# loopinf/SpotV2Net

Measured on NVIDIA B200. Metric: SpotV2Net GAT fwd+bwd graphs/sec (30-node, batch 4096), higher is better.
Workload: dtype f32

## Files before the change

spotv2net_b200/csrc/gemm.cuh:

```cuda
#pragma once
#include "common.cuh"

namespace spotv2 {

int sgemm_simt(bool a_kc, bool b_kc, int M, int N, int K, const float* A, int lda, const float* B,
               int ldb, float* C, int ldc, int splits, void* ws, size_t ws_bytes, cudaStream_t st);

struct BGemm {
  int M, N, K;
  const float* A;
  const float* B;
  float* C;
  int lda, ldb, ldc;
  int inner;
  long long a_o, a_i, b_o, b_i, c_o, c_i;
  int segs;
  long long a_s, b_s;
  float scale;
  const float* bias;
  long long bias_i;
  int vecA, vecB;
  int tensor_cores;
};
int bgemm_simt(bool a_kc, bool b_kc, BGemm g, int batches, cudaStream_t st);

inline int weight_grad_splits(int rows, int m, int n) {
  int base = (rows + 8191) / 8192;
  if (base < 1) base = 1;
  if (base > 32) base = 32;
  if (base == 1) return 1;
  const int tiles = ((m + 127) / 128) * ((n + 255) / 256);
  int best = base;
  double best_eff = 0.0;
  for (int s = base; s <= base + base / 4 + 1 && s <= 32; ++s) {
    const int items = tiles * s;
    const double eff = (double)items / (double)(((items + 147) / 148) * 148);
    if (eff > best_eff + 1e-9) { best = s; best_eff = eff; }
  }
  return best;
}

bool tc_gemm_supported(bool a_kc, bool b_kc, int M, int N, int K, const float* A_hi, int lda, const float* B_hi, int ldb);
int split_tf32(const float* src, float* hi, float* lo, size_t n, cudaStream_t st);
int gemm3x_tf32(bool a_kc, bool b_kc, int M, int N, int K, const float* A_hi, const float* A_lo, int lda,
                const float* B_hi, const float* B_lo, int ldb, float* C, int ldc, int splits, int bn,
                int kb_per_chunk, void* ws, size_t ws_bytes, cudaStream_t st);

struct F16Operand {
  const void* hi;
  const void* lo;
  int ld;
  const float* inv;
  int split_at;
};
struct PairOut {
  void* hi;
  void* lo;
  int ld;
  const float* scale;
// ... 20 lines not shown
```

spotv2net_b200/csrc/gemm_f16.cu:

```cuda
#include <cuda_fp16.h>
#include <stdio.h>
#include <stdlib.h>
#include <string.h>

#include <algorithm>

#include "gemm.cuh"
#include "tc.cuh"
#include "tma.cuh"

namespace spotv2 {

namespace {

constexpr int HBM_ = 128;
constexpr int HUMMA_K = 16;
constexpr int kHThreads = 384;
constexpr int kHEpiWarps = 8;

struct HParams {
  int M, N, K;
  int ldc;
  float* C;
  int m_tiles, n_tiles, splits, kb_per_split, kb_total, kb_per_chunk;
  size_t split_stride;
  const float* a_inv;
  const float* b_inv;
  int a_split, b_split;
  int scale_in_kernel;
  unsigned* amax_out;
  int amax_cols;
  int single;
  int pair_out;
  const float* out_scale;
  float* tail32;
  int tail_ld;
  int tma_store;
  int dbg;
};
#ifdef SPOTV2_BRINGUP
#define SPOTV2_DBG(p) ((p).dbg)
#else
#define SPOTV2_DBG(p) 0
#endif

template <int BN, int TBK, bool A_KM, bool B_KM>
struct HSmem {
  static constexpr int kAOp = HBM_ * TBK * 2;
  static constexpr int kBOp = BN * TBK * 2;
  static constexpr int kStage = 2 * kAOp + 2 * kBOp;
  static constexpr bool kWideEpi = (TBK == 32) && A_KM && B_KM;
  static constexpr int kStages = kWideEpi ? 3 : ((200 * 1024) / kStage > 6 ? 6 : (200 * 1024) / kStage);
  static constexpr int kBarOff = kStages * kStage;
  static constexpr int kEpiOff = kBarOff + 1024;
  static constexpr int kEpiWarpBytes = kWideEpi ? 8192 : 32 * 33 * 4;
  static constexpr int kBoxStride = kWideEpi ? 8192 : 4096;
  static constexpr int kPairBoxes = kWideEpi ? 4 : 2;
  static constexpr int kEpiBytes = kHEpiWarps * kEpiWarpBytes;
  static constexpr int kTotal = kEpiOff + kEpiBytes + 1024;
  static constexpr uint32_t kTxBytes = kStage;
};

template <int BN, int TBK, bool A_KM, bool B_KM>
__global__ void __launch_bounds__(kHThreads, 1)
gemm3x_f16_kernel(const __grid_constant__ CUtensorMap tmAh, const __grid_constant__ CUtensorMap tmAl,
                  const __grid_constant__ CUtensorMap tmBh, const __grid_constant__ CUtensorMap tmBl,
                  const __grid_constant__ CUtensorMap tmC, const HParams p) {
  using S = HSmem<BN, TBK, A_KM, B_KM>;
  constexpr int kStages = S::kStages;
  extern __shared__ unsigned char smem_dyn[];
  unsigned char* smem = reinterpret_cast<unsigned char*>((reinterpret_cast<uintptr_t>(smem_dyn) + 1023) & ~uintptr_t(1023));
  uint64_t* full = reinterpret_cast<uint64_t*>(smem + S::kBarOff);
  uint64_t* empty = full + kStages;
  uint64_t* tfull = empty + kStages;
  uint64_t* tempty = tfull + 2;
  uint32_t* tmem_slot = reinterpret_cast<uint32_t*>(tempty + 2);

  const int warp = threadIdx.x >> 5, lane = threadIdx.x & 31;
  const int total_tiles = p.m_tiles * p.n_tiles * p.splits;
  constexpr uint32_t kTmemCols = 2 * BN;

  if (warp == 0 && lane == 0) {
    prefetch_tmap(&tmAh); prefetch_tmap(&tmAl); prefetch_tmap(&tmBh); prefetch_tmap(&tmBl);
  }
  if (warp == 1 && lane == 0) {
    for (int s = 0; s < kStages; ++s) { mbar_init(&full[s], 1); mbar_init(&empty[s], 1); }
    for (int s = 0; s < 2; ++s) { mbar_init(&tfull[s], 1); mbar_init(&tempty[s], kHEpiWarps); }
    fence_mbar_init();
  }
  if (warp == 2) tmem_alloc(tmem_slot, kTmemCols);
  tc_fence_before();
  __syncthreads();
  tc_fence_after();
  const uint32_t tmem_base = *tmem_slot;

  auto tile_coords = [&](int tile, int& mt, int& nt, int& sp) {
    nt = tile % p.n_tiles;
    const int r = tile / p.n_tiles;
    mt = r % p.m_tiles;
    sp = r / p.m_tiles;
  };

  if (warp == 0) {
    if (elect_one()) {
      int stage = 0; uint32_t phase = 0;
      for (int tile = blockIdx.x; tile < total_tiles; tile += gridDim.x) {
        int mt, nt, sp; tile_coords(tile, mt, nt, sp);
        const int kb0 = sp * p.kb_per_split;
        const int kb1 = min(p.kb_total, kb0 + p.kb_per_split);
        for (int kb = kb0; kb < kb1; ++kb) {
          mbar_wait(&empty[stage], phase ^ 1);
          unsigned char* st = smem + stage * S::kStage;
          const bool lo = !p.single;
          mbar_expect_tx(&full[stage], lo ? S::kTxBytes : S::kTxBytes / 2);
          const int k = kb * TBK;
          if (A_KM) {
            tma_load_2d(st, &tmAh, k, mt * HBM_, &full[stage]);
            if (lo) tma_load_2d(st + S::kAOp, &tmAl, k, mt * HBM_, &full[stage]);
          } else {
#pragma unroll
            for (int blk = 0; blk < HBM_ / 64; ++blk) {
              tma_load_2d(st + blk * (TBK * 128), &tmAh, mt * HBM_ + blk * 64, k, &full[stage]);
              if (lo) tma_load_2d(st + S::kAOp + blk * (TBK * 128), &tmAl, mt * HBM_ + blk * 64, k, &full[stage]);
            }
          }
          unsigned char* sb = st + 2 * S::kAOp;
          if (B_KM) {
            tma_load_2d(sb, &tmBh, k, nt * BN, &full[stage]);
            if (lo) tma_load_2d(sb + S::kBOp, &tmBl, k, nt * BN, &full[stage]);
          } else {
#pragma unroll
            for (int blk = 0; blk < BN / 64; ++blk) {
              tma_load_2d(sb + blk * (TBK * 128), &tmBh, nt * BN + blk * 64, k, &full[stage]);
              if (lo) tma_load_2d(sb + S::kBOp + blk * (TBK * 128), &tmBl, nt * BN + blk * 64, k, &full[stage]);
            }
          }
          if (++stage == kStages) { stage = 0; phase ^= 1; }
        }
      }
    }
  } else if (warp == 1) {
    if (elect_one()) {
      constexpr uint32_t idesc = (1u << 4) | ((A_KM ? 0u : 1u) << 15) | ((B_KM ? 0u : 1u) << 16) |
                                 ((uint32_t)(BN >> 3) << 17) | ((uint32_t)(HBM_ >> 4) << 24);
      constexpr uint32_t k_sbo = 8 * TBK * 2, k_lt = (TBK == 64) ? 2 : 4;
      constexpr uint32_t a_lbo = A_KM ? 16 : TBK * 128, b_lbo = B_KM ? 16 : TBK * 128;
      constexpr uint32_t a_sbo = A_KM ? k_sbo : 1024, b_sbo = B_KM ? k_sbo : 1024;
      constexpr uint32_t a_lt = A_KM ? k_lt : 2, b_lt = B_KM ? k_lt : 2;
      constexpr uint32_t a_kstep = A_KM ? HUMMA_K * 2 : HUMMA_K * 128;
      constexpr uint32_t b_kstep = B_KM ? HUMMA_K * 2 : HUMMA_K * 128;
      int stage = 0; uint32_t phase = 0;
      uint32_t chunk_ctr = 0;
      for (int tile = blockIdx.x; tile < total_tiles; tile += gridDim.x) {
        int mt, nt, sp; tile_coords(tile, mt, nt, sp);
        const int kb0 = sp * p.kb_per_split;
        const int kb1 = min(p.kb_total, kb0 + p.kb_per_split);
        for (int kc = kb0; kc < kb1; kc += p.kb_per_chunk, ++chunk_ctr) {
          const int as = chunk_ctr & 1;
          mbar_wait(&tempty[as], ((chunk_ctr >> 1) & 1) ^ 1);
          tc_fence_after();
          const uint32_t d_tmem = tmem_base + (uint32_t)(as * BN);
          uint32_t accum = 0;
          const int kce = min(kb1, kc + p.kb_per_chunk);
          for (int kb = kc; kb < kce; ++kb) {
            mbar_wait(&full[stage], phase);
            tc_fence_after();
            const uint32_t sa = smem_u32(smem + stage * S::kStage);
            const uint32_t sb = sa + 2 * S::kAOp;
#pragma unroll
            for (int ks = 0; ks < TBK / HUMMA_K; ++ks) {
              const uint64_t ah = make_desc(sa + ks * a_kstep, a_lbo, a_sbo, a_lt);
              const uint64_t al = make_desc(sa + S::kAOp + ks * a_kstep, a_lbo, a_sbo, a_lt);
              const uint64_t bh = make_desc(sb + ks * b_kstep, b_lbo, b_sbo, b_lt);
              const uint64_t bl = make_desc(sb + S::kBOp + ks * b_kstep, b_lbo, b_sbo, b_lt);
              if (!p.single) {
                umma_f16(d_tmem, al, bh, idesc, accum);
                umma_f16(d_tmem, ah, bl, idesc, 1);
                accum = 1;
              }
              umma_f16(d_tmem, ah, bh, idesc, accum);
              accum = 1;
            }
            umma_commit(&empty[stage]);
            if (++stage == kStages) { stage = 0; phase ^= 1; }
          }
          umma_commit(&tfull[as]);
        }
      }
    }
  } else if (warp >= 4) {
    constexpr int HALF = BN / 2;
    const int q = warp & 3;
    const int ch = (warp - 4) >> 2;
    uint32_t chunk_ctr = 0;
    for (int tile = blockIdx.x; tile < total_tiles; tile += gridDim.x) {
      int mt, nt, sp; tile_coords(tile, mt, nt, sp);
      const int kb0 = sp * p.kb_per_split;
      const int kb1 = min(p.kb_total, kb0 + p.kb_per_split);
      float acc[HALF];
#pragma unroll
      for (int e = 0; e < HALF; ++e) acc[e] = 0.f;
      for (int kc = kb0; kc < kb1; kc += p.kb_per_chunk, ++chunk_ctr) {
        const int as = chunk_ctr & 1;
        mbar_wait(&tfull[as], (chunk_ctr >> 1) & 1);
        tc_fence_after();
        const uint32_t taddr = tmem_base + ((uint32_t)(q * 32) << 16) + (uint32_t)(as * BN + ch * HALF);
#pragma unroll
        for (int c0 = 0; c0 < HALF; c0 += 32) {
          uint32_t r[32];
          tmem_ld32(taddr + c0, r);
#pragma unroll
          if (!(SPOTV2_DBG(p) & 4))
#pragma unroll
            for (int e = 0; e < 32; ++e) acc[c0 + e] += __uint_as_float(r[e]);
          else acc[c0] += __uint_as_float(r[0]);
        }
        tc_fence_before();
        __syncwarp();
        if (lane == 0) mbar_arrive(&tempty[as]);
      }
      const int row = mt * HBM_ + q * 32 + lane;
      const int col0 = nt * BN + ch * HALF;
      float row_amax = 0.f;
      if (row < p.M && col0 < p.N && !(SPOTV2_DBG(p) & 2)) {
        if (p.scale_in_kernel) {
          const float ra = p.a_inv ? p.a_inv[row >= p.a_split ? 1 : 0] : 1.f;
          const float os0 = p.pair_out ? p.out_scale[0] : 1.f, os1 = p.pair_out ? p.out_scale[1] : 1.f;
          const float cb0 = ra * (p.b_inv ? p.b_inv[0] : 1.f) * os0, cb1 = ra * (p.b_inv ? p.b_inv[1] : 1.f) * os1;
#pragma unroll
          for (int e = 0; e < HALF; ++e) acc[e] *= (col0 + e >= p.b_split) ? cb1 : cb0;
        }
        if (p.amax_out) {
          float mx = 0.f;
#pragma unroll
          for (int e = 0; e < HALF; ++e)
            if (col0 + e < p.amax_cols) mx = fmaxf(mx, fabsf(acc[e]));
          row_amax = mx;
        }
      }
      if (p.pair_out && p.tail32 && row < p.M && col0 + HALF > p.b_split && col0 < p.N) {
        const float un = 1.f / p.out_scale[1];
        float* dst = p.tail32 + (size_t)row * p.tail_ld - p.b_split;
// ... 68 lines not shown
#pragma unroll
        for (int cc = 0; cc < HALF / 32; ++cc) {
#pragma unroll
          for (int j = 0; j < 32; ++j) stage[lane * 33 + j] = acc[cc * 32 + j];
          __syncwarp();
          const int col = col0 + cc * 32 + lane;
          if (col < p.N) {
#pragma unroll 8
            for (int rr = 0; rr < 32; ++rr)
              if (row_base + rr < p.M) cbase[(size_t)rr * p.ldc + col] = stage[rr * 33 + lane];
          }
          __syncwarp();
        }
      }
      if (p.amax_out) {
        for (int o = 16; o > 0; o >>= 1) row_amax = fmaxf(row_amax, __shfl_xor_sync(0xffffffffu, row_amax, o));
        if (lane == 0 && row_amax > 0.f) atomicMax(p.amax_out, __float_as_uint(row_amax));
      }
    }
  }

  if (warp >= 4 && lane == 0) asm volatile("cp.async.bulk.wait_group 0;" ::: "memory");
  tc_fence_before();
  __syncthreads();
  if (warp == 2) {
    tc_fence_after();
    tmem_dealloc(tmem_base, kTmemCols);
  }
}

__global__ void f16_splitk_reduce_kernel(const float* __restrict__ ws, int splits, size_t split_stride, int M, int N,
                                         float* __restrict__ C, int ldc, const float* __restrict__ a_inv, int a_split,
                                         const float* __restrict__ b_inv, int b_split) {
  const size_t idx = (size_t)blockIdx.x * blockDim.x + threadIdx.x;
  if (idx >= (size_t)M * N) return;
  float s = 0.f;
  for (int z = 0; z < splits; ++z) s += ws[(size_t)z * split_stride + idx];
  const int m = (int)(idx / N), n = (int)(idx - (size_t)m * N);
  const float f = (a_inv ? a_inv[m >= a_split ? 1 : 0] : 1.f) * (b_inv ? b_inv[n >= b_split ? 1 : 0] : 1.f);
  C[(size_t)m * ldc + n] = s * f;
}

template <int BN, int TBK, bool A_KM, bool B_KM>
int launch_h(const CUtensorMap& tAh, const CUtensorMap& tAl, const CUtensorMap& tBh, const CUtensorMap& tBl,
             const CUtensorMap& tC, const HParams& p, cudaStream_t st) {
  using S = HSmem<BN, TBK, A_KM, B_KM>;
  auto kern = gemm3x_f16_kernel<BN, TBK, A_KM, B_KM>;
  SPOTV2_CUDA_OK(cudaFuncSetAttribute(kern, cudaFuncAttributeMaxDynamicSharedMemorySize, S::kTotal));
  int grid = sm_count();
  const int total = p.m_tiles * p.n_tiles * p.splits;
  if (grid > total) grid = total;
  kern<<<grid, kHThreads, S::kTotal, st>>>(tAh, tAl, tBh, tBl, tC, p);
  SPOTV2_CUDA_OK(cudaGetLastError());
  return SPOTV2_OK;
}

__device__ __forceinline__ float scale_from_amax(float amax) {
  if (!(amax > 0.f) || !(amax < INFINITY)) return 1.f;
  int ex;
  frexpf(amax, &ex);
  return exp2f((float)(15 - ex));
}

__global__ void amax_kernel(const float* __restrict__ src, int rows, int cols, size_t ld, int split_dim, int split_at,
                            const float* __restrict__ pre2, int pre_split, unsigned* __restrict__ out_bits) {
  float m0 = 0.f, m1 = 0.f;
  const size_t total = (size_t)rows * cols;
  for (size_t idx = (size_t)blockIdx.x * blockDim.x + threadIdx.x; idx < total; idx += (size_t)gridDim.x * blockDim.x) {
    const int r = (int)(idx / cols), c = (int)(idx - (size_t)r * cols);
    float v = fabsf(src[(size_t)r * ld + c]);
    if (pre2) v *= pre2[r >= pre_split ? 1 : 0];
    const bool g1 = (split_dim == 0 ? r : c) >= split_at;
    if (g1) m1 = fmaxf(m1, v); else m0 = fmaxf(m0, v);
  }
  for (int o = 16; o > 0; o >>= 1) {
    m0 = fmaxf(m0, __shfl_xor_sync(0xffffffffu, m0, o));
// ... 250 lines not shown
    } else {
      if (int rc = launch_amax_flat(src, (size_t)r_split * cols, bits, st)) return rc;
      if (r_split < rows)
        if (int rc = launch_amax_flat(src + (size_t)r_split * cols, (size_t)(rows - r_split) * cols, bits + 1, st)) return rc;
    }
  } else {
    amax_kernel<<<blocks, 256, 0, st>>>(src, rows, cols, ld, split_dim, split_at, pre2, pre_split, bits);
  }
  const int vec4 = (cols % 4 == 0) && (ld % 4 == 0) && (ld16 % 4 == 0) && aligned16(src) &&
                   ((reinterpret_cast<uintptr_t>(hi) & 7) == 0) && ((reinterpret_cast<uintptr_t>(lo) & 7) == 0);
  if (vec4 && cols / 4 < 64)
    split_f16_narrow_kernel<<<(unsigned)std::min<size_t>(((size_t)rows * (cols / 4) + 255) / 256, (size_t)16 * 148), 256, 0, st>>>(
        src, rows, cols / 4, ld, split_dim, split_at, pre2, pre_split, static_cast<__half*>(hi), static_cast<__half*>(lo), ld16, blk);
  else if (vec4)
    split_f16_rows_kernel<<<std::min((rows + kSplitRows - 1) / kSplitRows, 32 * 148), 256, 0, st>>>(
        src, rows, cols / 4, ld, split_dim, split_at, pre2, pre_split, static_cast<__half*>(hi), static_cast<__half*>(lo), ld16, blk);
  else
    split_f16_kernel<<<blocks, 256, 0, st>>>(src, rows, cols, ld, split_dim, split_at, pre2, pre_split, 1.f,
                                             static_cast<__half*>(hi), static_cast<__half*>(lo), ld16, blk, 0);
  SPOTV2_CUDA_OK(cudaGetLastError());
  return SPOTV2_OK;
}

int gemm3x_f16(bool a_kc, bool b_kc, int M, int N, int K, const F16Operand& A, const F16Operand& B, float* C, int ldc,
               int splits, int bn, int kb_per_chunk, void* ws, size_t ws_bytes, cudaStream_t st, float* amax_out,
               int amax_cols, bool single, const PairOut* pair) {
  const int TBK = (bn & 16) ? 32 : 64;
  bn &= ~16;
  if (!tma_available()) return fail(SPOTV2_ERR_NO_DEVICE, "tensor-core GEMM: TMA descriptor encoding is not available");
  if (A.ld % 8 != 0 || B.ld % 8 != 0 || !aligned16(A.hi) || !aligned16(A.lo) || !aligned16(B.hi) || !aligned16(B.lo))
    return fail(SPOTV2_ERR_INVALID_ARG, "fp16 GEMM operands need 16-byte aligned bases and leading dimensions % 8 == 0");
  HParams p;
  p.M = M; p.N = N; p.K = K;
  p.m_tiles = (M + HBM_ - 1) / HBM_;
  p.n_tiles = (N + bn - 1) / bn;
  p.kb_total = (K + TBK - 1) / TBK;
  if (splits < 1) splits = 1;
  if (splits > p.kb_total) splits = p.kb_total;
  p.kb_per_split = (p.kb_total + splits - 1) / splits;
  p.splits = (p.kb_total + p.kb_per_split - 1) / p.kb_per_split;
  p.kb_per_chunk = kb_per_chunk < 1 ? 128 / TBK : kb_per_chunk;
  p.C = C; p.ldc = ldc; p.split_stride = 0;
  p.a_inv = A.inv; p.b_inv = B.inv; p.a_split = A.split_at; p.b_split = B.split_at;
  p.scale_in_kernel = 1;
  p.amax_out = reinterpret_cast<unsigned*>(amax_out);
  p.amax_cols = amax_cols;
  p.single = single ? 1 : 0;
  p.pair_out = 0; p.out_scale = nullptr; p.tail32 = nullptr; p.tail_ld = 0;
  if (pair) {
    if (splits > 1 || !pair->hi || !pair->scale || pair->ld % 8 != 0 || !aligned16(pair->hi) || (pair->lo && !aligned16(pair->lo)))
      return fail(SPOTV2_ERR_INVALID_ARG, "gemm3x_f16: pair output needs splits == 1, 16-byte aligned planes, ld %% 8 == 0 and a scale");
    p.pair_out = pair->lo ? 1 : 2;
    p.out_scale = pair->scale;
    p.tail32 = pair->tail32; p.tail_ld = pair->tail_ld;
  }
  p.dbg = 0;
#ifdef SPOTV2_BRINGUP
// ... 25 lines not shown
  if (pair) {
    const uint64_t plane_stride = pair->lo ? (uint64_t)((const __half*)pair->lo - (const __half*)pair->hi) : (uint64_t)M * pair->ld;
    if (pair->lo && ((const __half*)pair->lo <= (const __half*)pair->hi || plane_stride % 8 != 0))
      return fail(SPOTV2_ERR_INVALID_ARG, "gemm3x_f16: the lo plane must follow the hi plane at a multiple of 16 bytes");
    if ((rc = make_tmap3_f16(&tC, pair->hi, pair->lo ? 2 : 1, plane_stride, (uint64_t)M, (uint64_t)N, (uint64_t)pair->ld, 32, 32,
                             CU_TENSOR_MAP_SWIZZLE_64B)))
      return rc;
  } else if (aligned16(p.C) && p.ldc % 4 == 0 && (p.splits == 1 || p.split_stride % 4 == 0)) {
    if ((rc = make_tmap3(&tC, p.C, (uint64_t)p.splits, p.splits > 1 ? p.split_stride : (uint64_t)M * p.ldc, (uint64_t)M, (uint64_t)N,
                         (uint64_t)p.ldc, 16, 32, CU_TENSOR_MAP_SWIZZLE_64B)))
      return rc;
    p.tma_store = 1;
  }
  const CUtensorMapSwizzle kSw = TBK == 64 ? CU_TENSOR_MAP_SWIZZLE_128B : CU_TENSOR_MAP_SWIZZLE_64B;
  const CUtensorMapSwizzle mnSw = CU_TENSOR_MAP_SWIZZLE_128B;
  if (a_kc) {
    if ((rc = make_tmap_f16(&tAh, A.hi, M, K, A.ld, TBK, HBM_, kSw))) return rc;
    if ((rc = make_tmap_f16(&tAl, A.lo, M, K, A.ld, TBK, HBM_, kSw))) return rc;
  } else {
    if ((rc = make_tmap_f16(&tAh, A.hi, K, M, A.ld, 64, TBK, mnSw))) return rc;
    if ((rc = make_tmap_f16(&tAl, A.lo, K, M, A.ld, 64, TBK, mnSw))) return rc;
  }
  if (b_kc) {
    if ((rc = make_tmap_f16(&tBh, B.hi, N, K, B.ld, TBK, bn, kSw))) return rc;
    if ((rc = make_tmap_f16(&tBl, B.lo, N, K, B.ld, TBK, bn, kSw))) return rc;
  } else {
    if ((rc = make_tmap_f16(&tBh, B.hi, K, N, B.ld, 64, TBK, mnSw))) return rc;
    if ((rc = make_tmap_f16(&tBl, B.lo, K, N, B.ld, 64, TBK, mnSw))) return rc;
  }
#define SPOTV2_H(BN_, TBK_, AK, BK_) rc = launch_h<BN_, TBK_, AK, BK_>(tAh, tAl, tBh, tBl, tC, p, st)
#define SPOTV2_H_MAJ(BN_, TBK_)                            \
  do {                                                     \
    if (a_kc && b_kc) SPOTV2_H(BN_, TBK_, true, true);     \
    else if (a_kc) SPOTV2_H(BN_, TBK_, true, false);       \
    else if (b_kc) SPOTV2_H(BN_, TBK_, false, true);       \
    else SPOTV2_H(BN_, TBK_, false, false);                \
  } while (0)
  if (bn == 256 && TBK == 64) SPOTV2_H_MAJ(256, 64);
  else if (bn == 256 && TBK == 32) SPOTV2_H_MAJ(256, 32);
  else if (bn == 128 && TBK == 64) SPOTV2_H_MAJ(128, 64);
  else return fail(SPOTV2_ERR_INVALID_ARG, "bn must be 128, 256 or 256+16");
#undef SPOTV2_H_MAJ
#undef SPOTV2_H
  if (rc) return rc;
  if (p.splits > 1) {
    const size_t total = (size_t)M * N;
    f16_splitk_reduce_kernel<<<(unsigned)((total + 255) / 256), 256, 0, st>>>(p.C, p.splits, p.split_stride, M, N, C, ldc,
                                                                             A.inv, A.split_at, B.inv, B.split_at);
    SPOTV2_CUDA_OK(cudaGetLastError());
  }
  return SPOTV2_OK;
}

// ... 2 lines not shown
```

spotv2net_b200/csrc/proj.cu:

```cuda
#include "attn_bwd.cuh"
#include "gemm.cuh"

using namespace spotv2;

namespace {

constexpr int kNone = 0x7fffffff;

struct ProjShape {
  int rows, n_aug, HC, F, ldp, ldf16, ldp16;
};

ProjShape shape_of(const spotv2_gat_desc* d) {
  const int n_aug = n_aug_of(d);
  return {d->B * d->N, n_aug, d->H * head_pitch_of(d), d->F, d->ldp, ld16_of(d->F), ld16_of(n_aug)};
}

bool use_tc(const spotv2_gat_desc* d) { return d->gemm_algo != 1; }
bool single_product(const spotv2_gat_desc* d) { return d->gemm_algo == 3; }

struct Carver {
  unsigned char* p;
  size_t left;
  void* take(size_t bytes) {
// ... 1 lines not shown
    if (!p || bytes > left) return nullptr;
    void* r = p;
    p += bytes;
    left -= bytes;
    return r;
  }
};

size_t pair_bytes(size_t rows, size_t ld16) { return 2 * round_up(rows * ld16 * 2, 256); }

}

extern "C" int32_t spotv2_gat_ld16(int32_t cols) { return ld16_of(cols); }
extern "C" int32_t spotv2_diag_weight_grad_splits(int32_t rows, int32_t m, int32_t n) { return weight_grad_splits(rows, m, n); }

extern "C" int spotv2_gat_workspace_bytes(const spotv2_gat_desc* d, size_t* proj_fwd,
                                          size_t* attn_bwd, size_t* proj_bwd) {
  if (int rc = check_desc(d)) return rc;
  const ProjShape s = shape_of(d);
  const bool tc = use_tc(d);
  if (proj_fwd) *proj_fwd = 1024 + (tc ? pair_bytes(s.rows, s.ldf16) + pair_bytes(s.n_aug, s.ldf16) : 0);
  if (attn_bwd) *attn_bwd = attn_bwd_ws_bytes(d) + 256;
  if (proj_bwd) {
    const int splits = weight_grad_splits(s.rows, s.n_aug, s.F);
    size_t w = round_up((size_t)splits * s.n_aug * s.F * sizeof(float), 256) + 1024;
    if (tc) w += pair_bytes(s.rows, s.ldp16) + pair_bytes(s.rows, s.ldf16) + pair_bytes(s.n_aug, s.ldf16);
    *proj_bwd = w;
  }
  return SPOTV2_OK;
}

extern "C" int spotv2_gat_attn_fwd_workspace_bytes(const spotv2_gat_desc* d, size_t* attn_fwd) {
  if (int rc = check_desc(d)) return rc;
  SPOTV2_REQUIRE(attn_fwd, "attn_fwd_workspace_bytes: null pointer");
  *attn_fwd = attn_large_fwd_ws_bytes(d);
  return SPOTV2_OK;
}

extern "C" int spotv2_gat_edge_terms_bytes(const spotv2_gat_desc* d, size_t* bytes) {
  if (int rc = check_desc(d)) return rc;
  SPOTV2_REQUIRE(bytes, "edge_terms_bytes: null pointer");
  const size_t per_graph = (size_t)d->H * d->N * (d->N > 32 ? (size_t)d->N : (size_t)kEdgeTermNS);
  *bytes = d->Fe > 0 ? (size_t)d->B * per_graph * sizeof(float) : 0;
  return SPOTV2_OK;
}

extern "C" int spotv2_gat_uses_tensor_cores(const spotv2_gat_desc* d) {
// ... 52 lines not shown
  cudaStream_t st = as_stream(stream);
  Carver c{static_cast<unsigned char*>(ws), ws ? ws_bytes : 0};
  float* wblk = static_cast<float*>(c.take(2 * kScaleBlockFloats * sizeof(float)));
  void* wh = c.take((size_t)s.n_aug * s.ldf16 * 2);
  void* wl = c.take((size_t)s.n_aug * s.ldf16 * 2);
  if (!wblk || !wh || !wl) return fail(SPOTV2_ERR_WORKSPACE, "proj_fwd_pair: workspace too small (%zu B)", ws_bytes);
  if (int rc = w_pair_and_out_scale(W_aug, s.n_aug, s.F, s.HC, wh, wl, s.ldf16, wblk, x_scale, p_scale, st)) return rc;
  F16Operand A{x_hi, x_lo, s.ldf16, x_scale + 2, kNone}, B{wh, wl, s.ldf16, wblk + 2, s.HC};
  PairOut out{P_hi, single_product(d) ? nullptr : P_lo_or_null, s.ldp16, p_scale + 4, sd, 2 * d->H};
  return gemm3x_f16(true, true, s.rows, s.n_aug, s.F, A, B, nullptr, 0, 1, 256 + 16, 0, nullptr, 0, st, nullptr, 0, single_product(d),
                    &out);
}

extern "C" int spotv2_proj_bwd_weight(const spotv2_gat_desc* d, const float* x, const void* x_hi, const void* x_lo,
                                      const float* x_scale, const float* dP_aug, const void* dP_hi, const void* dP_lo,
                                      const float* dp_scale, float* dW_aug, void* ws, size_t ws_bytes, void* stream) {
  if (int rc = check_desc(d)) return rc;
  SPOTV2_REQUIRE((x || x_hi) && dW_aug && (dP_aug || dP_hi), "proj_bwd_weight: null pointer");
  if (d->p_format == 1 && single_product(d) && dP_hi && !dP_lo) dP_lo = dP_hi;
  SPOTV2_REQUIRE(d->p_format == 0 || (dP_hi && dP_lo && dp_scale && x_hi && x_lo && x_scale),
                 "proj_bwd_weight: p_format 1 takes x and dP as pairs");
  const ProjShape s = shape_of(d);
  cudaStream_t st = as_stream(stream);
  const int splits = weight_grad_splits(s.rows, s.n_aug, s.F);
  if (!use_tc(d)) {
    SPOTV2_REQUIRE(dP_aug, "proj_bwd_weight: the CUDA-core path takes the fp32 dP_aug");
    return sgemm_simt(false, false, s.n_aug, s.F, s.rows, dP_aug, s.ldp, x, s.F, dW_aug, s.F, splits, ws, ws_bytes, st);
  }
  Carver c{static_cast<unsigned char*>(ws), ws ? ws_bytes : 0};
  float* blk = static_cast<float*>(c.take(2 * kScaleBlockFloats * sizeof(float)));
  const bool have_x = x_hi && x_lo && x_scale, have_p = dP_hi && dP_lo && dp_scale;
  void* ph = have_p ? const_cast<void*>(dP_hi) : c.take((size_t)s.rows * s.ldp16 * 2);
  void* pl = have_p ? const_cast<void*>(dP_lo) : c.take((size_t)s.rows * s.ldp16 * 2);
  void* xh = have_x ? const_cast<void*>(x_hi) : c.take((size_t)s.rows * s.ldf16 * 2);
  void* xl = have_x ? const_cast<void*>(x_lo) : c.take((size_t)s.rows * s.ldf16 * 2);
  if (!blk || !ph || !pl || !xh || !xl) return fail(SPOTV2_ERR_WORKSPACE, "proj_bwd_weight: workspace too small (%zu B)", ws_bytes);
  const float *ps = dp_scale, *xs = x_scale;
  if (!have_p) {
    SPOTV2_REQUIRE(dP_aug, "proj_bwd_weight: dP_aug or the complete pair (dP_hi, dP_lo, dp_scale)");
    if (int rc = split_f16(dP_aug, s.rows, s.n_aug, s.ldp, 1, s.HC, nullptr, 0, ph, pl, s.ldp16, blk, st)) return rc;
    ps = blk;
  }
  if (!have_x) {
    if (int rc = split_f16(x, s.rows, s.F, s.F, 0, kNone, nullptr, 0, xh, xl, s.ldf16, blk + kScaleBlockFloats, st)) return rc;
    xs = blk + kScaleBlockFloats;
  }
  F16Operand A{ph, pl, s.ldp16, ps + 2, s.HC}, B{xh, xl, s.ldf16, xs + 2, kNone};
// ... 38 lines not shown
```

spotv2net_b200/csrc/tc.cuh:

```cuda
#pragma once
#include "common.cuh"

namespace spotv2 {

__device__ __forceinline__ void mbar_arrive(uint64_t* bar) {
  asm volatile("mbarrier.arrive.shared::cta.b64 _, [%0];" ::"r"(smem_u32(bar)) : "memory");
}
__device__ __forceinline__ void tc_fence_before() { asm volatile("tcgen05.fence::before_thread_sync;" ::: "memory"); }
__device__ __forceinline__ void tc_fence_after() { asm volatile("tcgen05.fence::after_thread_sync;" ::: "memory"); }
__device__ __forceinline__ void tmem_alloc(uint32_t* smem_dst, uint32_t ncols) {
  asm volatile("tcgen05.alloc.cta_group::1.sync.aligned.shared::cta.b32 [%0], %1;" ::"r"(smem_u32(smem_dst)), "r"(ncols)
               : "memory");
  asm volatile("tcgen05.relinquish_alloc_permit.cta_group::1.sync.aligned;" ::: "memory");
}
__device__ __forceinline__ void tmem_dealloc(uint32_t taddr, uint32_t ncols) {
  asm volatile("tcgen05.dealloc.cta_group::1.sync.aligned.b32 %0, %1;" ::"r"(taddr), "r"(ncols) : "memory");
}
__device__ __forceinline__ void umma_tf32(uint32_t tmem_d, uint64_t adesc, uint64_t bdesc, uint32_t idesc, uint32_t accum) {
  asm volatile(
      "{\n\t.reg .pred p;\n\tsetp.ne.b32 p, %4, 0;\n\t"
      "tcgen05.mma.cta_group::1.kind::tf32 [%0], %1, %2, %3, p;\n\t}" ::"r"(tmem_d),
      "l"(adesc), "l"(bdesc), "r"(idesc), "r"(accum)
      : "memory");
}
__device__ __forceinline__ void umma_f16(uint32_t tmem_d, uint64_t adesc, uint64_t bdesc, uint32_t idesc, uint32_t accum) {
  asm volatile(
      "{\n\t.reg .pred p;\n\tsetp.ne.b32 p, %4, 0;\n\t"
      "tcgen05.mma.cta_group::1.kind::f16 [%0], %1, %2, %3, p;\n\t}" ::"r"(tmem_d),
      "l"(adesc), "l"(bdesc), "r"(idesc), "r"(accum)
      : "memory");
}
__device__ __forceinline__ void umma_commit(uint64_t* bar) {
  asm volatile("tcgen05.commit.cta_group::1.mbarrier::arrive::one.shared::cluster.b64 [%0];" ::"r"(smem_u32(bar)) : "memory");
}
__device__ __forceinline__ void tmem_ld32(uint32_t taddr, uint32_t (&r)[32]) {
  asm volatile(
      "tcgen05.ld.sync.aligned.32x32b.x32.b32 {%0,%1,%2,%3,%4,%5,%6,%7,%8,%9,%10,%11,%12,%13,%14,%15,%16,%17,%18,%19,%20,%21,"
      "%22,%23,%24,%25,%26,%27,%28,%29,%30,%31}, [%32];"
      : "=r"(r[0]), "=r"(r[1]), "=r"(r[2]), "=r"(r[3]), "=r"(r[4]), "=r"(r[5]), "=r"(r[6]), "=r"(r[7]), "=r"(r[8]),
        "=r"(r[9]), "=r"(r[10]), "=r"(r[11]), "=r"(r[12]), "=r"(r[13]), "=r"(r[14]), "=r"(r[15]), "=r"(r[16]),
        "=r"(r[17]), "=r"(r[18]), "=r"(r[19]), "=r"(r[20]), "=r"(r[21]), "=r"(r[22]), "=r"(r[23]), "=r"(r[24]),
        "=r"(r[25]), "=r"(r[26]), "=r"(r[27]), "=r"(r[28]), "=r"(r[29]), "=r"(r[30]), "=r"(r[31])
      : "r"(taddr));
  asm volatile("tcgen05.wait::ld.sync.aligned;" ::: "memory");
}
__device__ __forceinline__ bool elect_one() {
  uint32_t pred;
  asm volatile(
      "{\n\t.reg .pred P;\n\t.reg .b32 R;\n\telect.sync R|P, 0xffffffff;\n\tselp.u32 %0, 1, 0, P;\n\t}"
      : "=r"(pred));
  return pred != 0;
}

__device__ __forceinline__ uint64_t make_desc(uint32_t smem_addr, uint32_t lbo_bytes, uint32_t sbo_bytes,
                                              uint32_t layout_type) {
  uint64_t d = 0;
  d |= (uint64_t)((smem_addr >> 4) & 0x3FFF);
// ... 9 lines not shown
```

spotv2net_b200/csrc/tma.cuh:

```cuda
#pragma once
#include <cuda.h>

#include "common.cuh"

namespace spotv2 {

typedef CUresult (*EncodeTiledFn)(CUtensorMap*, CUtensorMapDataType, cuuint32_t, void*, const cuuint64_t*,
                                  const cuuint64_t*, const cuuint32_t*, const cuuint32_t*, CUtensorMapInterleave,
                                  CUtensorMapSwizzle, CUtensorMapL2promotion, CUtensorMapFloatOOBfill);

inline EncodeTiledFn encode_fn() {
  static EncodeTiledFn fn = nullptr;
  if (fn) return fn;
  void* sym = nullptr;
  cudaDriverEntryPointQueryResult qres;
  if (cudaGetDriverEntryPoint("cuTensorMapEncodeTiled", &sym, cudaEnableDefault, &qres) != cudaSuccess ||
      qres != cudaDriverEntryPointSuccess)
    return nullptr;
  fn = reinterpret_cast<EncodeTiledFn>(sym);
  return fn;
}

inline bool tma_available() { return encode_fn() != nullptr; }

// ... 82 lines not shown
__device__ __forceinline__ void tma_store_wait_read() { asm volatile("cp.async.bulk.wait_group.read 0;" ::: "memory"); }
__device__ __forceinline__ void tma_load_4d(void* smem_dst, const CUtensorMap* tm, int c0, int c1, int c2, int c3, uint64_t* bar) {
  asm volatile(
      "cp.async.bulk.tensor.4d.shared::cluster.global.mbarrier::complete_tx::bytes [%0], [%1, {%3, %4, %5, %6}], [%2];" ::"r"(
          smem_u32(smem_dst)),
      "l"(tm), "r"(smem_u32(bar)), "r"(c0), "r"(c1), "r"(c2), "r"(c3)
      : "memory");
}
__device__ __forceinline__ void tma_load_4d_hint(void* smem_dst, const CUtensorMap* tm, int c0, int c1, int c2, int c3, uint64_t* bar,
                                                 uint64_t hint) {
  asm volatile(
      "cp.async.bulk.tensor.4d.shared::cluster.global.mbarrier::complete_tx::bytes.L2::cache_hint [%0], [%1, {%3, %4, %5, %6}], "
      "[%2], %7;" ::"r"(smem_u32(smem_dst)),
      "l"(tm), "r"(smem_u32(bar)), "r"(c0), "r"(c1), "r"(c2), "r"(c3), "l"(hint)
      : "memory");
}
__device__ __forceinline__ void tma_load_2d(void* smem_dst, const CUtensorMap* tm, int c0, int c1, uint64_t* bar) {
  asm volatile(
      "cp.async.bulk.tensor.2d.shared::cluster.global.mbarrier::complete_tx::bytes [%0], [%1, {%3, %4}], [%2];" ::"r"(
          smem_u32(smem_dst)),
      "l"(tm), "r"(smem_u32(bar)), "r"(c0), "r"(c1)
      : "memory");
}
__device__ __forceinline__ void tma_load_2d_hint(void* smem_dst, const CUtensorMap* tm, int c0, int c1, uint64_t* bar,
                                                 uint64_t hint) {
  asm volatile(
      "cp.async.bulk.tensor.2d.shared::cluster.global.mbarrier::complete_tx::bytes.L2::cache_hint [%0], [%1, {%3, %4}], "
      "[%2], %5;" ::"r"(smem_u32(smem_dst)),
      "l"(tm), "r"(smem_u32(bar)), "r"(c0), "r"(c1), "l"(hint)
      : "memory");
}
__device__ __forceinline__ void prefetch_tmap(const CUtensorMap* tm) {
  asm volatile("prefetch.tensormap [%0];" ::"l"(tm) : "memory");
}

}
```

Measured before the change: 581,700.

## Run fp16 split GEMM as 2-CTA cluster UMMA pairs

Converts the fp16 3-product tcgen05 GEMM to cta_group::2 when not in single-product mode. Two CTAs form a cluster that shares a 256-row M tile, each loads half of the B tile, and rank 0 issues paired MMAs with multicast commits and paired TMEM allocation. Weight-grad split selection now counts tiles and the number of resident cluster pairs. The aim is to halve per-CTA B operand traffic and smem use and to raise MMA efficiency. In exchange it adds cluster synchronisation, a smaller stage ring, and timeout-trap waits in the hot loops.

```diff
diff --git a/spotv2net_b200/csrc/gemm.cuh b/spotv2net_b200/csrc/gemm.cuh
--- a/spotv2net_b200/csrc/gemm.cuh
+++ b/spotv2net_b200/csrc/gemm.cuh
@@ -24,17 +24,21 @@
 };
 int bgemm_simt(bool a_kc, bool b_kc, BGemm g, int batches, cudaStream_t st);
 
-inline int weight_grad_splits(int rows, int m, int n) {
+int gemm3x_f16_resident_pairs();
+
+inline int weight_grad_splits(int rows, int m, int n, bool pair_tiles = true) {
   int base = (rows + 8191) / 8192;
   if (base < 1) base = 1;
   if (base > 32) base = 32;
   if (base == 1) return 1;
-  const int tiles = ((m + 127) / 128) * ((n + 255) / 256);
+  const int tile_m = pair_tiles ? 256 : 128;
+  const int tiles = ((m + tile_m - 1) / tile_m) * ((n + 255) / 256);
+  const int pairs = pair_tiles ? gemm3x_f16_resident_pairs() : sm_count();
   int best = base;
   double best_eff = 0.0;
   for (int s = base; s <= base + base / 4 + 1 && s <= 32; ++s) {
     const int items = tiles * s;
-    const double eff = (double)items / (double)(((items + 147) / 148) * 148);
+    const double eff = (double)items / (double)(((items + pairs - 1) / pairs) * pairs);
     if (eff > best_eff + 1e-9) { best = s; best_eff = eff; }
   }
   return best;
diff --git a/spotv2net_b200/csrc/gemm_f16.cu b/spotv2net_b200/csrc/gemm_f16.cu
--- a/spotv2net_b200/csrc/gemm_f16.cu
+++ b/spotv2net_b200/csrc/gemm_f16.cu
@@ -22,7 +22,7 @@
   int M, N, K;
   int ldc;
   float* C;
-  int m_tiles, n_tiles, splits, kb_per_split, kb_total, kb_per_chunk;
+  int pm_tiles, n_tiles, splits, kb_per_split, kb_total, kb_per_chunk;
   size_t split_stride;
   const float* a_inv;
   const float* b_inv;
@@ -44,13 +44,14 @@
 #define SPOTV2_DBG(p) 0
 #endif
 
-template <int BN, int TBK, bool A_KM, bool B_KM>
+template <int BN, int TBK, bool A_KM, bool B_KM, int CTAS>
 struct HSmem {
   static constexpr int kAOp = HBM_ * TBK * 2;
-  static constexpr int kBOp = BN * TBK * 2;
+  static constexpr int kBOp = (BN / CTAS) * TBK * 2;
   static constexpr int kStage = 2 * kAOp + 2 * kBOp;
   static constexpr bool kWideEpi = (TBK == 32) && A_KM && B_KM;
-  static constexpr int kStages = kWideEpi ? 3 : ((200 * 1024) / kStage > 6 ? 6 : (200 * 1024) / kStage);
+  static constexpr int kRingBytes = CTAS == 2 ? 160 * 1024 : 200 * 1024, kMaxStages = CTAS == 2 ? 4 : 6;
+  static constexpr int kStages = kWideEpi ? 3 : (kRingBytes / kStage > kMaxStages ? kMaxStages : kRingBytes / kStage);
   static constexpr int kBarOff = kStages * kStage;
   static constexpr int kEpiOff = kBarOff + 1024;
   static constexpr int kEpiWarpBytes = kWideEpi ? 8192 : 32 * 33 * 4;
@@ -58,15 +59,32 @@
   static constexpr int kPairBoxes = kWideEpi ? 4 : 2;
   static constexpr int kEpiBytes = kHEpiWarps * kEpiWarpBytes;
   static constexpr int kTotal = kEpiOff + kEpiBytes + 1024;
-  static constexpr uint32_t kTxBytes = kStage;
+  static constexpr uint32_t kTxBytes = CTAS * kStage;
 };
 
-template <int BN, int TBK, bool A_KM, bool B_KM>
+enum { kWaitFull = 0, kWaitEmpty, kWaitTempty, kWaitPeerEmpty };
+__device__ __noinline__ void gemm_wait_report(int id, uint32_t parity) {
+  const char* const names[] = {"full (operands landed)", "empty (stage consumed)", "tempty (accumulator drained)",
+                               "empty at exit (last stage released)"};
+  printf("gemm3x_f16: wait on %s timed out (block %d rank %u thread %d parity %u)\n", names[id], (int)blockIdx.x,
+         cluster_ctarank(), (int)threadIdx.x, parity);
+}
+__device__ __forceinline__ void hwait(uint64_t* bar, uint32_t parity, int id) {
+  for (int spin = 0; spin < 16; ++spin)
+    if (mbar_try_wait(bar, parity)) return;
+  const long long t0 = clock64();
+  while (!mbar_try_wait(bar, parity)) {
+    __nanosleep(64);
+    if (clock64() - t0 > 4000000000LL) { gemm_wait_report(id, parity); __trap(); }
+  }
+}
+
+template <int BN, int TBK, bool A_KM, bool B_KM, int CTAS>
 __global__ void __launch_bounds__(kHThreads, 1)
 gemm3x_f16_kernel(const __grid_constant__ CUtensorMap tmAh, const __grid_constant__ CUtensorMap tmAl,
                   const __grid_constant__ CUtensorMap tmBh, const __grid_constant__ CUtensorMap tmBl,
                   const __grid_constant__ CUtensorMap tmC, const HParams p) {
-  using S = HSmem<BN, TBK, A_KM, B_KM>;
+  using S = HSmem<BN, TBK, A_KM, B_KM, CTAS>;
   constexpr int kStages = S::kStages;
   extern __shared__ unsigned char smem_dyn[];
   unsigned char* smem = reinterpret_cast<unsigned char*>((reinterpret_cast<uintptr_t>(smem_dyn) + 1023) & ~uintptr_t(1023));
@@ -77,7 +95,9 @@
   uint32_t* tmem_slot = reinterpret_cast<uint32_t*>(tempty + 2);
 
   const int warp = threadIdx.x >> 5, lane = threadIdx.x & 31;
-  const int total_tiles = p.m_tiles * p.n_tiles * p.splits;
+  const uint32_t rank = CTAS == 2 ? cluster_ctarank() : 0;
+  const int pair_id = blockIdx.x / CTAS, num_pairs = gridDim.x / CTAS;
+  const int total_items = p.pm_tiles * p.n_tiles * p.splits;
   constexpr uint32_t kTmemCols = 2 * BN;
 
   if (warp == 0 && lane == 0) {
@@ -85,64 +105,89 @@
   }
   if (warp == 1 && lane == 0) {
     for (int s = 0; s < kStages; ++s) { mbar_init(&full[s], 1); mbar_init(&empty[s], 1); }
-    for (int s = 0; s < 2; ++s) { mbar_init(&tfull[s], 1); mbar_init(&tempty[s], kHEpiWarps); }
+    for (int s = 0; s < 2; ++s) { mbar_init(&tfull[s], 1); mbar_init(&tempty[s], CTAS * kHEpiWarps); }
     fence_mbar_init();
   }
-  if (warp == 2) tmem_alloc(tmem_slot, kTmemCols);
-  tc_fence_before();
-  __syncthreads();
+  if constexpr (CTAS == 2) {
+    if (warp == 2) tmem_alloc_pair(tmem_slot, kTmemCols);
+    tc_fence_before();
+    cluster_sync();
+  } else {
+    if (warp == 2) tmem_alloc(tmem_slot, kTmemCols);
+    tc_fence_before();
+    __syncthreads();
+  }
   tc_fence_after();
   const uint32_t tmem_base = *tmem_slot;
 
-  auto tile_coords = [&](int tile, int& mt, int& nt, int& sp) {
-    nt = tile % p.n_tiles;
-    const int r = tile / p.n_tiles;
-    mt = r % p.m_tiles;
-    sp = r / p.m_tiles;
+  auto tile_coords = [&](int item, int& mt, int& nt, int& sp) {
+    nt = item % p.n_tiles;
+    const int r = item / p.n_tiles;
+    mt = CTAS * (r % p.pm_tiles) + (int)rank;
+    sp = r / p.pm_tiles;
   };
 
   if (warp == 0) {
     if (elect_one()) {
+      const uint32_t full_leader = CTAS == 2 ? mapa_shared(full, 0) : 0;
       int stage = 0; uint32_t phase = 0;
-      for (int tile = blockIdx.x; tile < total_tiles; tile += gridDim.x) {
-        int mt, nt, sp; tile_coords(tile, mt, nt, sp);
+      for (int item = pair_id; item < total_items; item += num_pairs) {
+        int mt, nt, sp; tile_coords(item, mt, nt, sp);
         const int kb0 = sp * p.kb_per_split;
         const int kb1 = min(p.kb_total, kb0 + p.kb_per_split);
+        const int n0 = nt * BN + (int)rank * (BN / CTAS);
         for (int kb = kb0; kb < kb1; ++kb) {
-          mbar_wait(&empty[stage], phase ^ 1);
+          hwait(&empty[stage], phase ^ 1, kWaitEmpty);
           unsigned char* st = smem + stage * S::kStage;
           const bool lo = !p.single;
-          mbar_expect_tx(&full[stage], lo ? S::kTxBytes : S::kTxBytes / 2);
+          const uint32_t fb = full_leader + stage * (uint32_t)sizeof(uint64_t);
+          if (rank == 0) mbar_expect_tx(&full[stage], lo ? S::kTxBytes : S::kTxBytes / 2);
+          auto tma_load = [&](void* dst, const CUtensorMap* tm, int c0, int c1) {
+            if constexpr (CTAS == 2) tma_load_2d_pair(dst, tm, c0, c1, fb);
+            else tma_load_2d(dst, tm, c0, c1, &full[stage]);
+          };
           const int k = kb * TBK;
           if (A_KM) {
-            tma_load_2d(st, &tmAh, k, mt * HBM_, &full[stage]);
-            if (lo) tma_load_2d(st + S::kAOp, &tmAl, k, mt * HBM_, &full[stage]);
+            tma_load(st, &tmAh, k, mt * HBM_);
+            if (lo) tma_load(st + S::kAOp, &tmAl, k, mt * HBM_);
           } else {
 #pragma unroll
             for (int blk = 0; blk < HBM_ / 64; ++blk) {
-              tma_load_2d(st + blk * (TBK * 128), &tmAh, mt * HBM_ + blk * 64, k, &full[stage]);
-              if (lo) tma_load_2d(st + S::kAOp + blk * (TBK * 128), &tmAl, mt * HBM_ + blk * 64, k, &full[stage]);
+              tma_load(st + blk * (TBK * 128), &tmAh, mt * HBM_ + blk * 64, k);
+              if (lo) tma_load(st + S::kAOp + blk * (TBK * 128), &tmAl, mt * HBM_ + blk * 64, k);
             }
           }
           unsigned char* sb = st + 2 * S::kAOp;
           if (B_KM) {
-            tma_load_2d(sb, &tmBh, k, nt * BN, &full[stage]);
-            if (lo) tma_load_2d(sb + S::kBOp, &tmBl, k, nt * BN, &full[stage]);
+            tma_load(sb, &tmBh, k, n0);
+            if (lo) tma_load(sb + S::kBOp, &tmBl, k, n0);
           } else {
 #pragma unroll
-            for (int blk = 0; blk < BN / 64; ++blk) {
-              tma_load_2d(sb + blk * (TBK * 128), &tmBh, nt * BN + blk * 64, k, &full[stage]);
-              if (lo) tma_load_2d(sb + S::kBOp + blk * (TBK * 128), &tmBl, nt * BN + blk * 64, k, &full[stage]);
+            for (int blk = 0; blk < BN / CTAS / 64; ++blk) {
+              tma_load(sb + blk * (TBK * 128), &tmBh, n0 + blk * 64, k);
+              if (lo) tma_load(sb + S::kBOp + blk * (TBK * 128), &tmBl, n0 + blk * 64, k);
             }
           }
           if (++stage == kStages) { stage = 0; phase ^= 1; }
         }
       }
+      for (int s = 0; s < kStages; ++s) {
+        hwait(&empty[stage], phase ^ 1, kWaitPeerEmpty);
+        if (++stage == kStages) { stage = 0; phase ^= 1; }
+      }
     }
   } else if (warp == 1) {
-    if (elect_one()) {
+    if (rank == 0 && elect_one()) {
+      auto mma = [&](uint32_t d, uint64_t a, uint64_t b, uint32_t idesc, uint32_t acc) {
+        if constexpr (CTAS == 2) umma_f16_pair(d, a, b, idesc, acc);
+        else umma_f16(d, a, b, idesc, acc);
+      };
+      auto commit = [&](uint64_t* bar) {
+        if constexpr (CTAS == 2) umma_commit_pair(bar, 0x3);
+        else umma_commit(bar);
+      };
       constexpr uint32_t idesc = (1u << 4) | ((A_KM ? 0u : 1u) << 15) | ((B_KM ? 0u : 1u) << 16) |
-                                 ((uint32_t)(BN >> 3) << 17) | ((uint32_t)(HBM_ >> 4) << 24);
+                                 ((uint32_t)(BN >> 3) << 17) | ((uint32_t)((CTAS * HBM_) >> 4) << 24);
       constexpr uint32_t k_sbo = 8 * TBK * 2, k_lt = (TBK == 64) ? 2 : 4;
       constexpr uint32_t a_lbo = A_KM ? 16 : TBK * 128, b_lbo = B_KM ? 16 : TBK * 128;
       constexpr uint32_t a_sbo = A_KM ? k_sbo : 1024, b_sbo = B_KM ? k_sbo : 1024;
@@ -151,19 +196,19 @@
       constexpr uint32_t b_kstep = B_KM ? HUMMA_K * 2 : HUMMA_K * 128;
       int stage = 0; uint32_t phase = 0;
       uint32_t chunk_ctr = 0;
-      for (int tile = blockIdx.x; tile < total_tiles; tile += gridDim.x) {
-        int mt, nt, sp; tile_coords(tile, mt, nt, sp);
+      for (int item = pair_id; item < total_items; item += num_pairs) {
+        int mt, nt, sp; tile_coords(item, mt, nt, sp);
         const int kb0 = sp * p.kb_per_split;
         const int kb1 = min(p.kb_total, kb0 + p.kb_per_split);
         for (int kc = kb0; kc < kb1; kc += p.kb_per_chunk, ++chunk_ctr) {
           const int as = chunk_ctr & 1;
-          mbar_wait(&tempty[as], ((chunk_ctr >> 1) & 1) ^ 1);
+          hwait(&tempty[as], ((chunk_ctr >> 1) & 1) ^ 1, kWaitTempty);
           tc_fence_after();
           const uint32_t d_tmem = tmem_base + (uint32_t)(as * BN);
           uint32_t accum = 0;
           const int kce = min(kb1, kc + p.kb_per_chunk);
           for (int kb = kc; kb < kce; ++kb) {
-            mbar_wait(&full[stage], phase);
+            hwait(&full[stage], phase, kWaitFull);
             tc_fence_after();
             const uint32_t sa = smem_u32(smem + stage * S::kStage);
             const uint32_t sb = sa + 2 * S::kAOp;
@@ -174,17 +219,17 @@
               const uint64_t bh = make_desc(sb + ks * b_kstep, b_lbo, b_sbo, b_lt);
               const uint64_t bl = make_desc(sb + S::kBOp + ks * b_kstep, b_lbo, b_sbo, b_lt);
               if (!p.single) {
-                umma_f16(d_tmem, al, bh, idesc, accum);
-                umma_f16(d_tmem, ah, bl, idesc, 1);
+                mma(d_tmem, al, bh, idesc, accum);
+                mma(d_tmem, ah, bl, idesc, 1);
                 accum = 1;
               }
-              umma_f16(d_tmem, ah, bh, idesc, accum);
+              mma(d_tmem, ah, bh, idesc, accum);
               accum = 1;
             }
-            umma_commit(&empty[stage]);
+            commit(&empty[stage]);
             if (++stage == kStages) { stage = 0; phase ^= 1; }
           }
-          umma_commit(&tfull[as]);
+          commit(&tfull[as]);
         }
       }
     }
@@ -192,9 +237,10 @@
     constexpr int HALF = BN / 2;
     const int q = warp & 3;
     const int ch = (warp - 4) >> 2;
+    const uint32_t tempty_leader = CTAS == 2 ? mapa_shared(tempty, 0) : 0;
     uint32_t chunk_ctr = 0;
-    for (int tile = blockIdx.x; tile < total_tiles; tile += gridDim.x) {
-      int mt, nt, sp; tile_coords(tile, mt, nt, sp);
+    for (int item = pair_id; item < total_items; item += num_pairs) {
+      int mt, nt, sp; tile_coords(item, mt, nt, sp);
       const int kb0 = sp * p.kb_per_split;
       const int kb1 = min(p.kb_total, kb0 + p.kb_per_split);
       float acc[HALF];
@@ -217,7 +263,10 @@
         }
         tc_fence_before();
         __syncwarp();
-        if (lane == 0) mbar_arrive(&tempty[as]);
+        if (lane == 0) {
+          if constexpr (CTAS == 2) mbar_arrive_cluster(tempty_leader + as * (uint32_t)sizeof(uint64_t));
+          else mbar_arrive(&tempty[as]);
+        }
       }
       const int row = mt * HBM_ + q * 32 + lane;
       const int col0 = nt * BN + ch * HALF;
@@ -332,10 +381,18 @@
 
   if (warp >= 4 && lane == 0) asm volatile("cp.async.bulk.wait_group 0;" ::: "memory");
   tc_fence_before();
-  __syncthreads();
-  if (warp == 2) {
-    tc_fence_after();
-    tmem_dealloc(tmem_base, kTmemCols);
+  if constexpr (CTAS == 2) {
+    cluster_sync();
+    if (warp == 2) {
+      tc_fence_after();
+      tmem_dealloc_pair(tmem_base, kTmemCols);
+    }
+  } else {
+    __syncthreads();
+    if (warp == 2) {
+      tc_fence_after();
+      tmem_dealloc(tmem_base, kTmemCols);
+    }
   }
 }
 
@@ -352,16 +409,59 @@
 }
 
 template <int BN, int TBK, bool A_KM, bool B_KM>
+int resident_pairs_h() {
+  constexpr int CTAS = 2;
+  static int cached[64] = {0};
+  int dev = 0;
+  if (cudaGetDevice(&dev) != cudaSuccess) return 0;
+  if (dev >= 0 && dev < 64 && cached[dev]) return cached[dev];
+  using S = HSmem<BN, TBK, A_KM, B_KM, CTAS>;
+  auto kern = gemm3x_f16_kernel<BN, TBK, A_KM, B_KM, CTAS>;
+  if (cudaFuncSetAttribute(kern, cudaFuncAttributeMaxDynamicSharedMemorySize, S::kTotal) != cudaSuccess) return 0;
+  cudaLaunchAttribute attr;
+  attr.id = cudaLaunchAttributeClusterDimension;
+  attr.val.clusterDim.x = CTAS; attr.val.clusterDim.y = 1; attr.val.clusterDim.z = 1;
+  cudaLaunchConfig_t cfg = {};
+  cfg.gridDim = dim3(CTAS * sm_count());
+  cfg.blockDim = dim3(kHThreads);
+  cfg.dynamicSmemBytes = S::kTotal;
+  cfg.attrs = &attr;
+  cfg.numAttrs = 1;
+  int n = 0;
+  if (cudaOccupancyMaxActiveClusters(&n, kern, &cfg) != cudaSuccess || n <= 0) return 0;
+  if (dev >= 0 && dev < 64) cached[dev] = n;
+  return n;
+}
+
+template <int BN, int TBK, bool A_KM, bool B_KM, int CTAS>
 int launch_h(const CUtensorMap& tAh, const CUtensorMap& tAl, const CUtensorMap& tBh, const CUtensorMap& tBl,
              const CUtensorMap& tC, const HParams& p, cudaStream_t st) {
-  using S = HSmem<BN, TBK, A_KM, B_KM>;
-  auto kern = gemm3x_f16_kernel<BN, TBK, A_KM, B_KM>;
-  SPOTV2_CUDA_OK(cudaFuncSetAttribute(kern, cudaFuncAttributeMaxDynamicSharedMemorySize, S::kTotal));
-  int grid = sm_count();
-  const int total = p.m_tiles * p.n_tiles * p.splits;
-  if (grid > total) grid = total;
-  kern<<<grid, kHThreads, S::kTotal, st>>>(tAh, tAl, tBh, tBl, tC, p);
-  SPOTV2_CUDA_OK(cudaGetLastError());
+  using S = HSmem<BN, TBK, A_KM, B_KM, CTAS>;
+  auto kern = gemm3x_f16_kernel<BN, TBK, A_KM, B_KM, CTAS>;
+  int slots;
+  if constexpr (CTAS == 2) {
+    slots = resident_pairs_h<BN, TBK, A_KM, B_KM>();
+    if (slots <= 0) {
+      cudaGetLastError();
+      return fail(SPOTV2_ERR_CUDA, "gemm3x_f16: no cluster of two CTAs with %d B of shared memory fits on this device", S::kTotal);
+    }
+  } else {
+    SPOTV2_CUDA_OK(cudaFuncSetAttribute(kern, cudaFuncAttributeMaxDynamicSharedMemorySize, S::kTotal));
+    slots = sm_count();
+  }
+  const int total = p.pm_tiles * p.n_tiles * p.splits;
+  if (slots > total) slots = total;
+  cudaLaunchAttribute attr;
+  attr.id = cudaLaunchAttributeClusterDimension;
+  attr.val.clusterDim.x = CTAS; attr.val.clusterDim.y = 1; attr.val.clusterDim.z = 1;
+  cudaLaunchConfig_t cfg = {};
+  cfg.gridDim = dim3(CTAS * slots);
+  cfg.blockDim = dim3(kHThreads);
+  cfg.dynamicSmemBytes = S::kTotal;
+  cfg.stream = st;
+  cfg.attrs = &attr;
+  cfg.numAttrs = CTAS == 2 ? 1 : 0;
+  SPOTV2_CUDA_OK(cudaLaunchKernelEx(&cfg, kern, tAh, tAl, tBh, tBl, tC, p));
   return SPOTV2_OK;
 }
 
@@ -658,6 +758,13 @@
   return SPOTV2_OK;
 }
 
+int gemm3x_f16_resident_pairs() {
+  const int n = resident_pairs_h<256, 32, false, false>();
+  if (n > 0) return n;
+  cudaGetLastError();
+  return sm_count() / 2;
+}
+
 int gemm3x_f16(bool a_kc, bool b_kc, int M, int N, int K, const F16Operand& A, const F16Operand& B, float* C, int ldc,
                int splits, int bn, int kb_per_chunk, void* ws, size_t ws_bytes, cudaStream_t st, float* amax_out,
                int amax_cols, bool single, const PairOut* pair) {
@@ -668,7 +775,8 @@
     return fail(SPOTV2_ERR_INVALID_ARG, "fp16 GEMM operands need 16-byte aligned bases and leading dimensions % 8 == 0");
   HParams p;
   p.M = M; p.N = N; p.K = K;
-  p.m_tiles = (M + HBM_ - 1) / HBM_;
+  const int ctas = single ? 1 : 2;
+  p.pm_tiles = (M + ctas * HBM_ - 1) / (ctas * HBM_);
   p.n_tiles = (N + bn - 1) / bn;
   p.kb_total = (K + TBK - 1) / TBK;
   if (splits < 1) splits = 1;
@@ -740,13 +848,14 @@
     if ((rc = make_tmap_f16(&tAl, A.lo, K, M, A.ld, 64, TBK, mnSw))) return rc;
   }
   if (b_kc) {
-    if ((rc = make_tmap_f16(&tBh, B.hi, N, K, B.ld, TBK, bn, kSw))) return rc;
-    if ((rc = make_tmap_f16(&tBl, B.lo, N, K, B.ld, TBK, bn, kSw))) return rc;
+    if ((rc = make_tmap_f16(&tBh, B.hi, N, K, B.ld, TBK, bn / ctas, kSw))) return rc;
+    if ((rc = make_tmap_f16(&tBl, B.lo, N, K, B.ld, TBK, bn / ctas, kSw))) return rc;
   } else {
     if ((rc = make_tmap_f16(&tBh, B.hi, K, N, B.ld, 64, TBK, mnSw))) return rc;
     if ((rc = make_tmap_f16(&tBl, B.lo, K, N, B.ld, 64, TBK, mnSw))) return rc;
   }
-#define SPOTV2_H(BN_, TBK_, AK, BK_) rc = launch_h<BN_, TBK_, AK, BK_>(tAh, tAl, tBh, tBl, tC, p, st)
+#define SPOTV2_H(BN_, TBK_, AK, BK_) \
+  rc = single ? launch_h<BN_, TBK_, AK, BK_, 1>(tAh, tAl, tBh, tBl, tC, p, st) : launch_h<BN_, TBK_, AK, BK_, 2>(tAh, tAl, tBh, tBl, tC, p, st)
 #define SPOTV2_H_MAJ(BN_, TBK_)                            \
   do {                                                     \
     if (a_kc && b_kc) SPOTV2_H(BN_, TBK_, true, true);     \
diff --git a/spotv2net_b200/csrc/proj.cu b/spotv2net_b200/csrc/proj.cu
--- a/spotv2net_b200/csrc/proj.cu
+++ b/spotv2net_b200/csrc/proj.cu
@@ -47,7 +47,7 @@
   if (proj_fwd) *proj_fwd = 1024 + (tc ? pair_bytes(s.rows, s.ldf16) + pair_bytes(s.n_aug, s.ldf16) : 0);
   if (attn_bwd) *attn_bwd = attn_bwd_ws_bytes(d) + 256;
   if (proj_bwd) {
-    const int splits = weight_grad_splits(s.rows, s.n_aug, s.F);
+    const int splits = weight_grad_splits(s.rows, s.n_aug, s.F, !single_product(d));
     size_t w = round_up((size_t)splits * s.n_aug * s.F * sizeof(float), 256) + 1024;
     if (tc) w += pair_bytes(s.rows, s.ldp16) + pair_bytes(s.rows, s.ldf16) + pair_bytes(s.n_aug, s.ldf16);
     *proj_bwd = w;
@@ -146,7 +146,7 @@
                  "proj_bwd_weight: p_format 1 takes x and dP as pairs");
   const ProjShape s = shape_of(d);
   cudaStream_t st = as_stream(stream);
-  const int splits = weight_grad_splits(s.rows, s.n_aug, s.F);
+  const int splits = weight_grad_splits(s.rows, s.n_aug, s.F, !single_product(d));
   if (!use_tc(d)) {
     SPOTV2_REQUIRE(dP_aug, "proj_bwd_weight: the CUDA-core path takes the fp32 dP_aug");
     return sgemm_simt(false, false, s.n_aug, s.F, s.rows, dP_aug, s.ldp, x, s.F, dW_aug, s.F, splits, ws, ws_bytes, st);
diff --git a/spotv2net_b200/csrc/tc.cuh b/spotv2net_b200/csrc/tc.cuh
--- a/spotv2net_b200/csrc/tc.cuh
+++ b/spotv2net_b200/csrc/tc.cuh
@@ -33,6 +33,45 @@
 __device__ __forceinline__ void umma_commit(uint64_t* bar) {
   asm volatile("tcgen05.commit.cta_group::1.mbarrier::arrive::one.shared::cluster.b64 [%0];" ::"r"(smem_u32(bar)) : "memory");
 }
+
+__device__ __forceinline__ uint32_t cluster_ctarank() {
+  uint32_t r;
+  asm volatile("mov.u32 %0, %%cluster_ctarank;" : "=r"(r));
+  return r;
+}
+__device__ __forceinline__ void cluster_sync() {
+  asm volatile("barrier.cluster.arrive.release.aligned;\n\tbarrier.cluster.wait.acquire.aligned;" ::: "memory");
+}
+__device__ __forceinline__ uint32_t mapa_shared(const void* p, uint32_t rank) {
+  uint32_t r;
+  asm volatile("mapa.shared::cluster.u32 %0, %1, %2;" : "=r"(r) : "r"(smem_u32(p)), "r"(rank));
+  return r;
+}
+__device__ __forceinline__ void mbar_arrive_cluster(uint32_t cluster_addr) {
+  asm volatile("mbarrier.arrive.release.cluster.shared::cluster.b64 _, [%0];" ::"r"(cluster_addr) : "memory");
+}
+__device__ __forceinline__ void tmem_alloc_pair(uint32_t* smem_dst, uint32_t ncols) {
+  asm volatile("tcgen05.alloc.cta_group::2.sync.aligned.shared::cta.b32 [%0], %1;" ::"r"(smem_u32(smem_dst)), "r"(ncols)
+               : "memory");
+  asm volatile("tcgen05.relinquish_alloc_permit.cta_group::2.sync.aligned;" ::: "memory");
+}
+__device__ __forceinline__ void tmem_dealloc_pair(uint32_t taddr, uint32_t ncols) {
+  asm volatile("tcgen05.dealloc.cta_group::2.sync.aligned.b32 %0, %1;" ::"r"(taddr), "r"(ncols) : "memory");
+}
+__device__ __forceinline__ void umma_f16_pair(uint32_t tmem_d, uint64_t adesc, uint64_t bdesc, uint32_t idesc, uint32_t accum) {
+  asm volatile(
+      "{\n\t.reg .pred p;\n\tsetp.ne.b32 p, %4, 0;\n\t"
+      "tcgen05.mma.cta_group::2.kind::f16 [%0], %1, %2, %3, p;\n\t}" ::"r"(tmem_d),
+      "l"(adesc), "l"(bdesc), "r"(idesc), "r"(accum)
+      : "memory");
+}
+__device__ __forceinline__ void umma_commit_pair(uint64_t* bar, uint16_t cta_mask) {
+  asm volatile("tcgen05.commit.cta_group::2.mbarrier::arrive::one.shared::cluster.multicast::cluster.b64 [%0], %1;" ::"r"(
+                   smem_u32(bar)),
+               "h"(cta_mask)
+               : "memory");
+}
+
 __device__ __forceinline__ void tmem_ld32(uint32_t taddr, uint32_t (&r)[32]) {
   asm volatile(
       "tcgen05.ld.sync.aligned.32x32b.x32.b32 {%0,%1,%2,%3,%4,%5,%6,%7,%8,%9,%10,%11,%12,%13,%14,%15,%16,%17,%18,%19,%20,%21,"
diff --git a/spotv2net_b200/csrc/tma.cuh b/spotv2net_b200/csrc/tma.cuh
--- a/spotv2net_b200/csrc/tma.cuh
+++ b/spotv2net_b200/csrc/tma.cuh
@@ -128,6 +128,13 @@
       "l"(tm), "r"(smem_u32(bar)), "r"(c0), "r"(c1)
       : "memory");
 }
+__device__ __forceinline__ void tma_load_2d_pair(void* smem_dst, const CUtensorMap* tm, int c0, int c1, uint32_t bar_cluster) {
+  asm volatile(
+      "cp.async.bulk.tensor.2d.cta_group::2.shared::cluster.global.mbarrier::complete_tx::bytes [%0], [%1, {%3, %4}], [%2];" ::"r"(
+          smem_u32(smem_dst)),
+      "l"(tm), "r"(bar_cluster), "r"(c0), "r"(c1)
+      : "memory");
+}
 __device__ __forceinline__ void tma_load_2d_hint(void* smem_dst, const CUtensorMap* tm, int c0, int c1, uint64_t* bar,
                                                  uint64_t hint) {
   asm volatile(
```

Measured after the change: 612,000 (median of 6 runs). +5.2%, better.
